# yimin-pan/hair-gs

Measured on AMD Instinct MI355X. Metric: train_iters_per_sec, higher is better.
Workload: dtype f32; 1 GPU; north_star: 100000 strand-Gaussians, 32 views @ 1920x1080, 1 view(s)/GPU/optimizer step (1 views/step), RGB+mask+orientation raster fwd+bwd + L1/DSSIM/mask/orientation/smoothness losses + Adam; gaussians=100000, views=32, width=1920, height=1080, parallelism=view-parallel x1, views_per_optimizer_step=1, forward_mode=async-capacity, dispatch=hip-graph replay, optimizer_steps_per_graph_launch=8, adam_in_backward_lanes=True, raster_passes_per_iter=1

## Files before the change

### hair-gs_amd/csrc/hgs_api.hip

```cpp
#include <stdarg.h>
#include <stdio.h>
#include <string.h>

#include "hgs_common.h"
#include "hgs_prologue.h"

static thread_local char g_err[512] = "";

void hgs_set_error(const char* fmt, ...) {
  va_list ap;
  va_start(ap, fmt);
  vsnprintf(g_err, sizeof(g_err), fmt, ap);
  va_end(ap);
}

#include <vector>
namespace {
struct ProfRec { hipEvent_t a, b; int id; };
bool g_prof_on = false;
std::vector<ProfRec> g_prof_log;
std::vector<hipEvent_t> g_prof_pool;
hipEvent_t g_prof_open = nullptr;
int g_prof_open_id = -1;
const char* kKernelNames[HGS_K_COUNT] = {"preprocess_fwd_kernel", "scan_kernel", "scatter_kernel", "sort_tiles_kernel",
// ... 215 lines not shown
    if (!fused_scan) { hgs_set_error("hgs_params_forward_preprocess: the scan must be the scatter kernel's (sizes beyond its limits)"); return 1; }
    HgsStrandFusion fu = fusion ? *fusion : HgsStrandFusion{};
    if (!(fu.smooth_pairs && fu.n_smooth > 0 && fu.smooth_partials)) fu.n_smooth = 0;
    if (hgs_launch_param_preprocess_fwd(s, a, g, im, radii, *params, fu)) return 1;
  } else if (hgs_launch_preprocess_fwd(s, a, g, im, radii)) return 1;
  if (!fused_scan && hgs_launch_scan(s, P, T, g, im, max_rendered, a.row_runs)) return 1;
  if (num_rendered_host) {
    uint32_t r = 0;
    HGS_CHECK_HIP(hipMemcpyAsync(&r, im.status, sizeof(uint32_t), hipMemcpyDeviceToHost, s));
    HGS_CHECK_HIP(hipStreamSynchronize(s));
    *num_rendered_host = (int)r;
  }
  return 0;
}

int hgs_forward_render(void* stream, int P, int W, int H, int R_capacity, int n_extra, int flags, const float* bg,
                       const float* colors_precomp, const float* extra, void* geom_buf, void* binning_buf, void* image_buf,
                       float* out_color) {
  hipStream_t s = (hipStream_t)stream;
  if (check_aligned(image_buf, "image_buf")) return 1;
  if (!bg || !out_color) { hgs_set_error("null bg/out_color"); return 1; }
  if (n_extra != 0 && n_extra != 4) { hgs_set_error("n_extra must be 0 or 4 (got %d)", n_extra); return 1; }
  if (n_extra && P > 0 && (!extra || ((size_t)extra & 15))) { hgs_set_error("extra colours must be a 16-byte aligned [P,4] array"); return 1; }
  if ((flags & HGS_RECORDS_PACKED) && (flags & HGS_RECORDS_LAZY)) { hgs_set_error("HGS_RECORDS_PACKED and HGS_RECORDS_LAZY exclude each other"); return 1; }
  const int channels = 3 + n_extra;
  HgsImage im;
  hgs_image_carve((char*)image_buf, (size_t)W, (size_t)H, im, nullptr);
  HgsGeom g = {};
  HgsBinning b = {};
  if (P > 0) {
    if (check_aligned(geom_buf, "geom_buf")) return 1;
    hgs_geom_carve((char*)geom_buf, (size_t)P, g, nullptr);
    if (R_capacity > 0) {
      if (check_aligned(binning_buf, "binning_buf")) return 1;
      hgs_binning_carve((char*)binning_buf, (size_t)R_capacity, b, nullptr, channels);
      b.grec = g.grec;
      const long long tiles = (long long)((W + HGS_TILE - 1) / HGS_TILE) * ((H + HGS_TILE - 1) / HGS_TILE);
      b.lazy = (flags & HGS_RECORDS_LAZY) ? 1 : (flags & HGS_RECORDS_PACKED) ? 0 : ((long long)R_capacity >= (long long)HGS_LAZY_MIN_MEAN_LIST * tiles ? 1 : 0);
    }
    const float* feat = colors_precomp ? colors_precomp : g.rgb;
    if (hgs_launch_scatter(s, P, W, H, R_capacity > 0 ? R_capacity : 0, feat, extra, n_extra, g, im, b)) return 1;
  }
  if (hgs_launch_sort_tiles(s, W, H, R_capacity > 0 ? R_capacity : 0, n_extra, g, im, b)) return 1;
  return hgs_launch_blend_fwd(s, W, H, R_capacity > 0 ? R_capacity : 0, channels, bg, im, b, out_color);
}

#define HGS_RR_AUTO_RATIO 8

static int backward_impl(void* stream, int P, int D, int M, int R, int W, int H, int n_extra, int flags, const float* bg,
                         const float* means3D, const float* shs, const float* colors_precomp, const float* scales,
                         float scale_modifier, const float* rotations, const float* cov3D_precomp, const float* viewmatrix,
                         const float* projmatrix, const float* campos, float tan_fovx, float tan_fovy, const int* radii,
                         const void* geom_buf, const void* binning_buf, const void* image_buf,
                         const float* const* dL_dpix_planes, void* scratch, float* dL_dextra, float* dL_dmeans2D, float* dL_dconic,
                         float* dL_dopacity, float* dL_dcolors, float* dL_dmeans3D, float* dL_dcov3D, float* dL_dsh,
                         float* dL_dscales, float* dL_drotations, const HgsParamBackward* pb,
                         const HgsBlockPlan* plan = nullptr) {
  hipStream_t s = (hipStream_t)stream;
  if (n_extra != 0 && n_extra != 4) { hgs_set_error("n_extra must be 0 or 4 (got %d)", n_extra); return 1; }
// ... 328 lines not shown
```

### hair-gs_amd/csrc/hgs_blend.hip

```cpp
#include "hgs_common.h"

__device__ unsigned long long* g_wg_trace_fwd = nullptr;
__device__ unsigned long long* g_wg_trace_bwd = nullptr;
#ifndef HGS_WG_TRACE
#define HGS_WG_TRACE 0
#endif
struct WgTrace {
#if HGS_WG_TRACE
  unsigned long long* buf;
  __device__ WgTrace(unsigned long long* b) : buf(b ? b + 8 * (size_t)blockIdx.x : nullptr) { mark(0); }
  __device__ void mark(int k) const { if (buf && threadIdx.x == 0) buf[k] = __builtin_amdgcn_s_memrealtime(); }
  __device__ void item(int tile, uint32_t seg, uint32_t nseg, uint32_t len) const {
    if (buf && threadIdx.x == 0) buf[6] = (unsigned long long)tile | (unsigned long long)seg << 24 | (unsigned long long)nseg << 32 | (unsigned long long)len << 40;
  }
  __device__ void count(int k, unsigned v) const { if (buf && (threadIdx.x & 63) == 0) atomicAdd(&buf[k], (unsigned long long)v); }
  __device__ ~WgTrace() { mark(7); }
#else
  __device__ WgTrace(unsigned long long*) {}
  __device__ void mark(int) const {}
  __device__ void item(int, uint32_t, uint32_t, uint32_t) const {}
  __device__ void count(int, unsigned) const {}
#endif
};

// ... 173 lines not shown
        process(rb, eb);
        if (__ballot(T > 0.f) == 0ull) m = 0ull;
        if (m == 0ull) break;
      }
    }
    if (b + 1 < nb) {
      if (threadIdx.x < REC_BATCH * REC4) recs[cur ^ 1][threadIdx.x] = stage;
      const uint32_t wave_alive = __ballot(T > 0.f) != 0 ? 1u : 0u;
      if (lane == 0) alive[cur ^ 1][wave] = wave_alive;
    }
  }
}

template <int C>
__global__ __launch_bounds__(HGS_BLOCK) __attribute__((amdgpu_waves_per_eu(8))) void blend_fwd_kernel(HgsImage im, HgsBinning bn, int W, int H, int gx, uint32_t Rcap,
                                                              const float* __restrict__ bg, float* __restrict__ out_color) {
  constexpr int REC4 = Chan<C>::REC4;
  __shared__ float4 recs[2][REC_BATCH * REC4];
  __shared__ uint32_t alive[2][4];
  __shared__ uint32_t s_flag;
  BlendItem it;
  if (!blend_item(im, Rcap, it)) return;
  const int tile = it.tile;
  WgTrace _trace(g_wg_trace_fwd);
  _trace.item(tile, it.seg, it.nseg, it.e - it.s);
  const int tx = tile % gx, ty = tile / gx;
  const int wave = threadIdx.x >> 6, lane = threadIdx.x & 63;
  const int px = tx * HGS_TILE + (wave & 1) * 8 + (lane & 7);
  const int py = ty * HGS_TILE + (wave >> 1) * 8 + (lane >> 3);
  const bool inside = px < W && py < H;
  const float pxf = (float)px, pyf = (float)py;
  const uint32_t list0 = it.range.x;
  float acc[C];
#pragma unroll
  for (int k = 0; k < C; k++) acc[k] = 0.f;
  uint32_t last = 0;
  const size_t pix = (size_t)py * W + px, HW = (size_t)H * W;

  if (!it.split) {
    float T = inside ? 1.f : -1.f;
    fwd_walk<C>(bn, it.lazy, list0, tx, ty, 0u, it.e, recs, alive, pxf, pyf, wave, lane, T, acc, last);
    uint32_t wmax = last;
#pragma unroll
    for (int d = 32; d >= 1; d >>= 1) wmax = max(wmax, (uint32_t)__shfl_xor((int)wmax, d, 64));
    if (lane == 0 && wmax) atomicMax(&im.tile_maxc[tile], wmax);
    if (inside) {
      T = fabsf(T);
      im.final_T[pix] = T;
      im.n_contrib[pix] = last;
#pragma unroll
      for (int k = 0; k < C; k++) out_color[k * HW + pix] = acc[k] + T * bg[k];
    }
    return;
  }

  if (it.nseg == 2u) {
    if (it.seg == 1u) return;
    const uint32_t n = it.range.y - it.range.x;
    float T = inside ? 1.f : -1.f;
    fwd_walk<C>(bn, it.lazy, list0, tx, ty, 0u, it.e, recs, alive, pxf, pyf, wave, lane, T, acc, last);
    const size_t slot1 = ((size_t)it.w + 1) * HGS_BLOCK + threadIdx.x;
    bn.seg_T[slot1] = fabsf(T);
#pragma unroll
    for (int k = 0; k < C; k++) { bn.seg_C[((size_t)it.w * C + k) * HGS_BLOCK + threadIdx.x] = acc[k]; acc[k] = 0.f; }
    fwd_walk<C>(bn, it.lazy, list0, tx, ty, it.e, n, recs, alive, pxf, pyf, wave, lane, T, acc, last);
#pragma unroll
    for (int k = 0; k < C; k++) {
      bn.seg_C[(((size_t)it.w + 1) * C + k) * HGS_BLOCK + threadIdx.x] = acc[k];
      acc[k] += bn.seg_C[((size_t)it.w * C + k) * HGS_BLOCK + threadIdx.x];
      bn.seg_C[((size_t)it.w * C + k) * HGS_BLOCK + threadIdx.x] = acc[k];
    }
    uint32_t wmax = last;
#pragma unroll
    for (int d = 32; d >= 1; d >>= 1) wmax = max(wmax, (uint32_t)__shfl_xor((int)wmax, d, 64));
    if (lane == 0 && wmax) atomicMax(&im.tile_maxc[tile], wmax);
    if (inside) {
      T = fabsf(T);
      im.final_T[pix] = T;
      im.n_contrib[pix] = last;
#pragma unroll
      for (int k = 0; k < C; k++) out_color[k * HW + pix] = acc[k] + T * bg[k];
    }
    return;
  }

  const size_t slot = (size_t)it.w * HGS_BLOCK + threadIdx.x;
  const size_t slot0 = slot - (size_t)it.seg * HGS_BLOCK;
  float T = inside ? 1.f : -1.f;
  fwd_walk<C>(bn, it.lazy, list0, tx, ty, it.s, it.e, recs, alive, pxf, pyf, wave, lane, T, acc, last);
  const float P = inside ? fmaxf(T, 0.f) : -1.f;
// ... 96 lines not shown
        v[j][k] = mh - j >= 0 ? hgs_ld_agent(&bn.seg_C[((w0 + (size_t)(mh - j)) * C + k) * HGS_BLOCK + threadIdx.x]) : 0.f;
#pragma unroll
    for (int j = 0; j < FG; j++)
      if (mh - j >= 0) {
#pragma unroll
        for (int k = 0; k < C; k++) {
          if ((uint32_t)(mh - j) <= lastseg) acc[k] += v[j][k];
          bn.seg_C[((w0 + (size_t)(mh - j)) * C + k) * HGS_BLOCK + threadIdx.x] = acc[k];
        }
      }
  }
  uint32_t wmax = inside ? nc : 0u;
#pragma unroll
  for (int d = 32; d >= 1; d >>= 1) wmax = max(wmax, (uint32_t)__shfl_xor((int)wmax, d, 64));
  if (lane == 0 && wmax) atomicMax(&im.tile_maxc[tile], wmax);
  if (inside) {
    im.final_T[pix] = Tfin;
    im.n_contrib[pix] = nc;
#pragma unroll
    for (int k = 0; k < C; k++) out_color[k * HW + pix] = acc[k] + Tfin * bg[k];
  }
}

template <int C> struct PixGrad { const float* plane[C]; };

template <int C, bool BLACK>
__global__ __launch_bounds__(HGS_BLOCK) __attribute__((amdgpu_waves_per_eu(HGS_BWD_WAVES))) void blend_bwd_kernel(HgsImage im, HgsBinning bn, int W, int H, int gx,
                                                              uint32_t Rcap, const float* __restrict__ bg,
                                                              PixGrad<C> dL_dpix, float* __restrict__ inst_grad, int tag_rows) {
  constexpr int REC4 = Chan<C>::REC4, NPART = Chan<C>::NPART, NREG = Chan<C>::NREG, NV = 4 * NREG, ROW = Chan<C>::ROW;
// ... 166 lines not shown

}

extern "C" int hgs_debug_set_wg_trace(void* device_buf_fwd, void* device_buf_bwd) {
  HGS_CHECK_HIP(hipMemcpyToSymbol(HIP_SYMBOL(g_wg_trace_fwd), &device_buf_fwd, sizeof(void*)));
  HGS_CHECK_HIP(hipMemcpyToSymbol(HIP_SYMBOL(g_wg_trace_bwd), &device_buf_bwd, sizeof(void*)));
  return 0;
}

static inline unsigned blend_grid(int T, const HgsBinning& b) {
  const unsigned cap = (unsigned)HGS_SPLIT_CAPACITY(T);
  return (unsigned)T + (b.seg_cap < cap ? b.seg_cap : cap);
}

int hgs_launch_blend_fwd(hipStream_t s, int W, int H, int Rcap, int channels, const float* bg, const HgsImage& im,
                         const HgsBinning& b, float* out_color) {
  const int gx = (W + HGS_TILE - 1) / HGS_TILE, gy = (H + HGS_TILE - 1) / HGS_TILE;
  {
    HgsProfScope _prof(s, HGS_K_BLEND_FWD);
    if (channels == 3)
      hipLaunchKernelGGL(blend_fwd_kernel<3>, dim3(blend_grid(gx * gy, b)), dim3(HGS_BLOCK), 0, s, im, b, W, H, gx,
                         (uint32_t)Rcap, bg, out_color);
    else
      hipLaunchKernelGGL(blend_fwd_kernel<7>, dim3(blend_grid(gx * gy, b)), dim3(HGS_BLOCK), 0, s, im, b, W, H, gx,
                         (uint32_t)Rcap, bg, out_color);
  }
  HGS_CHECK_LAUNCH();
  return 0;
}

int hgs_launch_blend_bwd(hipStream_t s, int W, int H, int Rcap, int channels, const float* bg, const HgsImage& im,
                         const HgsBinning& b, const float* const* dL_dpix_planes, float* inst_grad, int tag_rows) {
  const int gx = (W + HGS_TILE - 1) / HGS_TILE, gy = (H + HGS_TILE - 1) / HGS_TILE;
  {
    HgsProfScope _prof(s, HGS_K_BLEND_BWD);
    if (channels == 3) {
      PixGrad<3> pg;
      for (int k = 0; k < 3; k++) pg.plane[k] = dL_dpix_planes[k];
      if (bg) hipLaunchKernelGGL((blend_bwd_kernel<3, false>), dim3(blend_grid(gx * gy, b)), dim3(HGS_BLOCK), 0, s, im, b, W, H, gx,
                                 (uint32_t)Rcap, bg, pg, inst_grad, tag_rows);
// ... 15 lines not shown
```

### hair-gs_amd/csrc/hgs_common.h

```cpp
#pragma once
#include <hip/hip_runtime.h>
#include <stdint.h>
#include <stddef.h>

#include "../../include/hgs.h"

#define HGS_BLOCK 256
#define HGS_WAVE 64
#define HGS_ALIGN 256

struct HgsRect {
  uint16_t x0, y0, x1, y1;
  uint32_t off;
  uint32_t pad;
};

struct HgsGeom {
  float* depths; uint8_t* clamped; float2* means2D; float* cov3D; float4* conic_opacity; float* rgb;
  uint32_t* tiles_touched; uint32_t* point_offsets; HgsRect* rect; uint32_t* block_sums;
  float4* grec;
};
struct HgsImage {
  float* final_T; uint32_t* n_contrib; uint2* ranges; uint32_t* tile_count; uint32_t* tile_cursor;
  int32_t* tile_delta;
  uint32_t* tile_maxc; uint32_t* status; uint32_t* tile_order; uint32_t* wl_exchange;
  uint32_t tile_mask;
  uint32_t* tile_done; unsigned long long* tile_prog; unsigned long long* tile_sortprog; uint32_t* sort_items;
};
struct HgsBinning {
  uint64_t* keys; uint32_t* point_list; float4* packed; uint32_t* inv; uint64_t* keys_sorted;
  float* seg_P;
  float* seg_T;
  float* seg_Tout;
  uint32_t* seg_last;
  float* seg_C;
  uint32_t seg_cap;
  const float4* grec;
  int lazy;
};
#ifndef HGS_LAZY_MIN_MEAN_LIST
#define HGS_LAZY_MIN_MEAN_LIST 128
#endif
// ... 84 lines not shown
  const HgsImageZero z = hgs_image_zero_layout(T);
  im.tile_mask = (uint32_t)(Tp - 1);
  hgs_carve(cur, im.tile_count, T);         if (offs) offs[HGS_IMG_TILE_COUNT] = (char*)im.tile_count - base;
  uint32_t* const zr = im.tile_count;
  im.tile_delta = (int32_t*)(zr + z.delta);
  im.tile_cursor = zr + z.cursor;           if (offs) offs[HGS_IMG_TILE_CURSOR] = (char*)im.tile_cursor - base;
  im.tile_maxc = zr + z.maxc;               if (offs) offs[HGS_IMG_TILE_MAXC] = (char*)im.tile_maxc - base;
  im.tile_done = zr + z.done;
  im.status = zr + z.status;                if (offs) offs[HGS_IMG_STATUS] = (char*)im.status - base;
  im.tile_prog = (unsigned long long*)(zr + z.prog);
  im.tile_sortprog = (unsigned long long*)(zr + z.sortprog);
  cur = (char*)(zr + z.words);
  hgs_carve(cur, im.sort_items, T);
  hgs_carve(cur, im.tile_order, T + HGS_SPLIT_CAPACITY(T));  if (offs) offs[HGS_IMG_TILE_ORDER] = (char*)im.tile_order - base;
  hgs_carve(cur, im.wl_exchange, HGS_WL_EXCHANGE_WORDS);
  return hgs_align_up((size_t)(cur - base)) + HGS_ALIGN;
}
static inline size_t hgs_binning_carve(char* base, size_t R, HgsBinning& b, size_t* offs, int channels = 3) {
  char* cur = base;
  hgs_carve(cur, b.keys, R);                                  if (offs) offs[HGS_BIN_KEYS] = (char*)b.keys - base;
  hgs_carve(cur, b.point_list, R);                            if (offs) offs[HGS_BIN_POINT_LIST] = (char*)b.point_list - base;
  hgs_carve(cur, b.packed, R * (channels <= 3 ? HGS_PACKED_FLOATS / 4 : 4) + 4);  if (offs) offs[HGS_BIN_PACKED] = (char*)b.packed - base;
  hgs_carve(cur, b.inv, R);                                   if (offs) offs[HGS_BIN_INV] = (char*)b.inv - base;
  hgs_carve(cur, b.keys_sorted, R);                           if (offs) offs[HGS_BIN_KEYS_TMP] = (char*)b.keys_sorted - base;
  b.seg_cap = hgs_seg_capacity(R);
  hgs_carve(cur, b.seg_P, (size_t)b.seg_cap * 256);
  hgs_carve(cur, b.seg_T, (size_t)b.seg_cap * 256);
  hgs_carve(cur, b.seg_Tout, (size_t)b.seg_cap * 256);
  hgs_carve(cur, b.seg_last, (size_t)b.seg_cap * 256);
  hgs_carve(cur, b.seg_C, (size_t)b.seg_cap * 256 * (channels <= 3 ? 3 : 7));
// ... 83 lines not shown
};
#ifndef HGS_FUSED_SCAN_MAX_P
#define HGS_FUSED_SCAN_MAX_P 0x7FFFFFFF
#endif
#define HGS_FUSED_SCAN_MAX_T 8192
int hgs_launch_preprocess_fwd(hipStream_t s, const HgsFwdArgs& a, const HgsGeom& g, const HgsImage& im, int* radii);
int hgs_launch_param_preprocess_fwd(hipStream_t s, const HgsFwdArgs& a, const HgsGeom& g, const HgsImage& im, int* radii,
                                    const HgsParamForward& pf, const HgsStrandFusion& fusion);
int hgs_param_forward_check(int P, const HgsParamForward* pf, bool one_launch, const char* who);
int hgs_launch_scan(hipStream_t s, int P, int T, const HgsGeom& g, const HgsImage& im, unsigned int* max_rendered, int row_runs = 0);
int hgs_launch_scatter(hipStream_t s, int P, int W, int H, int Rcap, const float* features, const float* extra, int n_extra,
                       const HgsGeom& g, const HgsImage& im, const HgsBinning& b);
int hgs_launch_sort_tiles(hipStream_t s, int W, int H, int Rcap, int n_extra, const HgsGeom& g, const HgsImage& im,
                          const HgsBinning& b);
int hgs_launch_blend_fwd(hipStream_t s, int W, int H, int Rcap, int channels, const float* bg, const HgsImage& im,
                         const HgsBinning& b, float* out_color);
int hgs_launch_blend_bwd(hipStream_t s, int W, int H, int Rcap, int channels, const float* bg, const HgsImage& im,
                         const HgsBinning& b, const float* const* dL_dpix_planes, float* inst_grad, int tag_rows = 0);
struct HgsBwdArgs {
  int P, D, M, W, H;
  const float *means3D, *shs, *colors_precomp, *scales, *rotations, *cov3D_precomp;
  const float *viewmatrix, *projmatrix, *campos;
  float scale_modifier, tan_fovx, tan_fovy;
  const int* radii;
  float *dL_dmeans2D, *dL_dconic, *dL_dopacity, *dL_dcolors, *dL_dmeans3D, *dL_dcov3D, *dL_dsh, *dL_dscales,
      *dL_drotations;
  int n_extra;
  float* dL_dextra;
  const float* row_sums;
  const float* row_partials;
};
// ... 97 lines not shown
```

### hair-gs_amd/diff_gaussian_rasterization/_C.py

```python
import contextlib
import ctypes as C
import os

import torch

import hgs_runtime as rt

IMAGE_PREZEROED = 2
COUNT_ROW_RUNS = 4
TILE_CULL = 8
RECORDS_PACKED, RECORDS_LAZY = 16, 32
ROWS_INLINE, ROWS_REDUCE = 64, 128
_state = {"async": False, "slack": 1.5, "cap": 0, "dirty": False, "cap_used": None,
          "max_R": {}, "last_exact_R": 0, "last_counts_clean": False,
          "cull": None, "row_reduce": None, "lazy_records": None, "row_runs": None}


class HgsCapacityOverflow(RuntimeError):
    pass


def bucket_capacity(n):
    n = int(n)
    if n <= 16:
# ... 41 lines not shown
    was = _state["row_runs"]
    _state["row_runs"] = None if mode is None else bool(mode)
    return was


def _row_runs_flag(P, use_async):
    mode = _pinned(_state["row_runs"], "HGS_ROW_RUNS")
    if mode is None:
        mode = (_state["cap"] if use_async else _state["last_exact_R"]) >= 8 * P
    return COUNT_ROW_RUNS if (mode and P > 0) else 0


def set_async(enabled=True, slack=1.5):
    _state["async"], _state["slack"] = bool(enabled), float(slack)
    _state["dirty"], _state["cap_used"] = False, None


@contextlib.contextmanager
def async_mode(enabled, slack=None):
    saved = {k: _state[k] for k in ("async", "slack", "dirty", "cap_used")}
    _state["async"], _state["slack"] = bool(enabled), _state["slack"] if slack is None else float(slack)
    try:
        yield
    finally:
        _state.update(saved)


def capacity():
    return _state["cap"]

# ... 66 lines not shown
    return _forward(background, means3D, colors, opacity, scales, rotations, scale_modifier, cov3D_precomp, viewmatrix,
                    projmatrix, tan_fovx, tan_fovy, image_height, image_width, sh, degree, campos, prefiltered, debug,
                    None, False)


def rasterize_gaussians_culled(background, means3D, colors, opacity, scales, rotations, scale_modifier, cov3D_precomp,
                               viewmatrix, projmatrix, tan_fovx, tan_fovy, image_height, image_width, sh, degree, campos,
                               prefiltered, debug):
    return _forward(background, means3D, colors, opacity, scales, rotations, scale_modifier, cov3D_precomp, viewmatrix,
                    projmatrix, tan_fovx, tan_fovy, image_height, image_width, sh, degree, campos, prefiltered, debug,
                    None, True)


def rasterize_gaussians_multi(background7, means3D, colors, extra4, opacity, scales, rotations, scale_modifier,
                              cov3D_precomp, viewmatrix, projmatrix, tan_fovx, tan_fovy, image_height, image_width, sh,
                              degree, campos, prefiltered, debug, image_buffer=None, hair=None):
    return _forward(background7, means3D, colors, opacity, scales, rotations, scale_modifier, cov3D_precomp, viewmatrix,
                    projmatrix, tan_fovx, tan_fovy, image_height, image_width, sh, degree, campos, prefiltered, debug,
                    extra4, True, image_buffer, None, hair)


class _ParamSource:

    def __init__(self, kind, fusion, fill, fuse, **inputs):
        self.params, self.fusion, self.fill, self.fuse = rt.ParamForward(kind=kind), fusion, fill, bool(fuse)
        self.inputs = {k: rt.require_gpu_tensor(t, k, torch.int64) if k == "endpoint_pairs" else _f32(t, k) for k, t in inputs.items()}
        for k, t in self.inputs.items():
            setattr(self.params, k, rt.ptr(t))


class HairSource(_ParamSource):

    def __init__(self, endpoints, pairs, width, factor, opacity_raw, mask_raw, fusion=None, fill=None, fuse=True):
        super().__init__(rt.PARAMS_HAIR, fusion, fill, fuse, endpoints=endpoints, endpoint_pairs=pairs, width=width,
# ... 11 lines not shown
def will_fuse_hair(W, H):
    return (_state["async"] and _state["cap"] > 0 and os.environ.get("HGS_FUSE_PREPROCESS", "1") != "0"
            and ((int(W) + 15) // 16) * ((int(H) + 15) // 16) <= rt.FUSED_PREPROCESS_MAX_TILES)


def rasterize_gaussians_prezeroed(background, means3D, colors, opacity, scales, rotations, scale_modifier, cov3D_precomp,
                                  viewmatrix, projmatrix, tan_fovx, tan_fovy, image_height, image_width, sh, degree, campos,
                                  image_buffer, max_rendered=None, hair=None):
    return _forward(background, means3D, colors, opacity, scales, rotations, scale_modifier, cov3D_precomp, viewmatrix,
                    projmatrix, tan_fovx, tan_fovy, image_height, image_width, sh, degree, campos, False, False,
                    None, True, image_buffer, max_rendered, hair)


def _forward(background, means3D, colors, opacity, scales, rotations, scale_modifier, cov3D_precomp, viewmatrix,
             projmatrix, tan_fovx, tan_fovy, image_height, image_width, sh, degree, campos, prefiltered, debug, extra4,
             cull, image_buffer=None, max_rendered=None, hair=None):
    if means3D.ndim != 2 or means3D.shape[1] != 3:
        raise RuntimeError("means3D must have dimensions (num_points, 3)")
    L = rt.lib()
    means3D = rt.require_gpu_tensor(means3D, "means3D", torch.float32)
    dev = means3D.device
    P, H, W = means3D.shape[0], int(image_height), int(image_width)
    M = sh.shape[1] if (sh is not None and sh.numel() != 0) else 0
    n_ch = 3 if extra4 is None else 7
    extra_ = None if extra4 is None else rt.require_gpu_tensor(extra4, "extra4", torch.float32)
    out_color = torch.empty((n_ch, H, W), dtype=torch.float32, device=dev)
    radii = torch.empty((P,), dtype=torch.int32, device=dev)
    u8 = dict(dtype=torch.uint8, device=dev)
    geom = torch.empty((L.hgs_geom_bytes(P),), **u8)
    cull = _state["cull"] if _state["cull"] is not None else cull
    flags = int(bool(prefiltered)) | (TILE_CULL if cull else 0)
    if image_buffer is not None:
        if image_buffer.numel() != L.hgs_image_bytes(W, H) or image_buffer.dtype != torch.uint8 or image_buffer.device != dev:
            raise RuntimeError("image_buffer: need a uint8 tensor of hgs_image_bytes(W, H) on the inputs' device")
        img, flags = image_buffer, flags | IMAGE_PREZEROED
    else:
        img = torch.empty((L.hgs_image_bytes(W, H),), **u8)
    bg = _f32(background, "bg")
    colors_, opacity_, scales_, rots_, cov_, sh_ = (_f32(colors, "colors_precomp"), _f32(opacity, "opacities"),
                                                     _f32(scales, "scales"), _f32(rotations, "rotations"),
                                                     _f32(cov3D_precomp, "cov3D_precomp"), _f32(sh, "sh"))
# ... 25 lines not shown
            rt.check(L.hgs_forward_preprocess(stream, P, int(degree), M, W, H, rt.ptr(means3D), rt.ptr(sh_), rt.ptr(colors_),
                                              rt.ptr(opacity_), rt.ptr(scales_), float(scale_modifier), rt.ptr(rots_),
                                              rt.ptr(cov_), rt.ptr(view), rt.ptr(proj), rt.ptr(cam), float(tan_fovx),
                                              float(tan_fovy), flags, rt.ptr(geom), rt.ptr(img),
                                              rt.ptr(radii), None if use_async else C.addressof(n_host), mr_))
        if P > 0:
            _state["last_counts_clean"] = bool(use_async and ((W + 15) // 16) * ((H + 15) // 16) <= rt.FUSED_PREPROCESS_MAX_TILES)
        if use_async:
            R = _state["cap"]
        else:
            R = int(n_host.value)
            _state["last_exact_R"] = R
            if _state["async"]:
                raise_capacity(R)
        binning = torch.empty((L.hgs_binning_bytes(R, n_ch),), **u8)
        rt.check(L.hgs_forward_render(stream, P, W, H, R, n_ch - 3, _records_flags(), rt.ptr(bg), rt.ptr(colors_),
                                      rt.ptr(extra_), rt.ptr(geom), rt.ptr(binning), rt.ptr(img), rt.ptr(out_color)))
        if use_async and max_rendered is None:
            _mark_pending(R)
        if debug:
            torch.cuda.synchronize(dev)
    return R, out_color, radii, geom, binning, img


def _scratch(nbytes, dev):
    buf = torch.empty((nbytes,), dtype=torch.uint8, device=dev)
    if os.environ.get("HGS_POISON_SCRATCH") == "1" and nbytes >= 4:
        buf[:nbytes // 4 * 4].view(torch.float32).fill_(float("nan"))
    return buf


def _backward(n_extra, background, means3D, radii, colors, scales, rotations, scale_modifier, cov3D_precomp, viewmatrix,
# ... 81 lines not shown
```

### hair-gs_amd/hgs_runtime/__init__.py

```python
import ctypes as C
import os
import subprocess

import numpy as np

_PKG_ROOT = os.path.dirname(os.path.dirname(os.path.abspath(__file__)))
LIB_PATH = os.environ.get("HGS_LIB") or os.path.join(_PKG_ROOT, "libhgs.so")
CSRC = os.path.join(_PKG_ROOT, "csrc")
_lib = None

vp, ci, cf, sz = C.c_void_p, C.c_int, C.c_float, C.c_size_t

SIGNATURES = {
    "hgs_abi_version": (ci, []),
    "hgs_last_error": (C.c_char_p, []),
    "hgs_geom_bytes": (sz, [ci]),
    "hgs_image_bytes": (sz, [ci, ci]),
    "hgs_binning_bytes": (sz, [ci, ci]),
    "hgs_backward_scratch_bytes": (sz, [ci, ci, ci]),
    "hgs_forward_preprocess": (ci, [vp, ci, ci, ci, ci, ci, vp, vp, vp, vp, vp, cf, vp, vp, vp, vp, vp, cf, cf, ci,
                                    vp, vp, vp, vp, vp]),
    "hgs_forward_render": (ci, [vp, ci, ci, ci, ci, ci, ci, vp, vp, vp, vp, vp, vp, vp]),
    "hgs_backward": (ci, [vp, ci, ci, ci, ci, ci, ci, ci, ci, vp, vp, vp, vp, vp, cf, vp, vp, vp, vp, vp, cf, cf, vp, vp, vp,
                          vp, vp, vp, vp, vp, vp, vp, vp, vp, vp, vp, vp, vp]),
    "hgs_param_backward_bytes": (sz, []),
    "hgs_backward_multi_params": (ci, [vp, ci, ci, ci, ci, ci, ci, ci, vp, vp, vp, vp, vp, vp, vp, vp, cf, cf, vp, vp, vp, vp, vp,
                                       vp, vp, vp]),
    "hgs_block_plan_bytes": (sz, []),
    "hgs_backward_multi_params_planned": (ci, [vp, ci, ci, ci, ci, ci, ci, ci, vp, vp, vp, vp, vp, vp, vp, vp, cf, cf, vp, vp, vp, vp,
                                               vp, vp, vp, vp, vp]),
    "hgs_hair_endpoint_gather": (ci, [vp, ci, vp, vp, vp, vp, vp]),
    "hgs_mark_visible": (ci, [vp, ci, vp, vp, vp, vp]),
    "hgs_dist2_scratch_bytes": (sz, [ci]),
    "hgs_dist2": (ci, [vp, ci, vp, vp, vp, sz]),
    "hgs_ssim_l1_scratch_floats": (sz, [ci, ci, ci]),
    "hgs_ssim_l1_num_blocks": (ci, [ci, ci, ci]),
    "hgs_ssim_l1_forward": (ci, [vp, ci, ci, ci, vp, vp, vp, vp, vp]),
# ... 93 lines not shown
    "hgs_raster_count": (ci, [vp, ci, ci, ci, ci, vp, C.c_longlong, vp, ci, vp, vp, vp]),
    "hgs_raster_fill": (ci, [vp, ci, ci, ci, ci, vp, C.c_longlong, vp, ci, vp, vp, vp, vp, vp]),
    "hgs_raster_resolve": (ci, [vp, ci, ci, ci, ci, vp, vp, ci, vp, vp, vp, vp, vp, vp, vp, vp, vp, vp, vp]),
    "hgs_set_segment_policy": (ci, [ci, ci, ci]),
    "hgs_debug_set_wg_trace": (ci, [vp, vp]),
    "hgs_prof_enable": (ci, [ci]),
    "hgs_prof_bracket_overhead_ms": (C.c_double, []),
    "hgs_prof_collect": (ci, [vp, vp]),
    "hgs_prof_kernel_name": (C.c_char_p, [ci]),
    "hgs_geom_layout": (ci, [ci, vp]),
    "hgs_image_layout": (ci, [ci, ci, vp]),
    "hgs_binning_layout": (ci, [ci, vp]),
}
GEOM_FIELDS = ["depths", "clamped", "means2D", "cov3D", "conic_opacity", "rgb", "tiles_touched", "point_offsets", "rect",
               "block_sums"]
IMG_FIELDS = ["final_T", "n_contrib", "ranges", "tile_count", "tile_cursor", "tile_maxc", "status", "tile_order"]
BIN_FIELDS = ["keys", "point_list", "packed", "inv", "keys_sorted"]
PACKED_FLOATS = 12
INST_GRAD_FLOATS = 12


class HgsError(RuntimeError):
    pass


class ViewTargets(C.Structure):
    _fields_ = [("image", vp), ("float_mask", vp), ("orientation", vp), ("confidence", vp), ("mask", vp),
                ("viewmatrix", cf * 16), ("projmatrix", cf * 16), ("campos", cf * 3), ("mask_count", cf)]


class HeadParams(C.Structure):
# ... 301 lines not shown
```

### hair-gs_amd/hgs_runtime/strand_step.py

```python
import ctypes as C
import functools
import os
import math

import numpy as np
import torch

import hgs_runtime as rt
from hgs_runtime.fused import gaussian_window11

_SLOT_BYTES = C.sizeof(rt.ViewTargets)
_F_VIEW, _F_PROJ, _F_CAM = (rt.ViewTargets.viewmatrix.offset // 4, rt.ViewTargets.projmatrix.offset // 4,
                            rt.ViewTargets.campos.offset // 4)


class ViewTable:

    def __init__(self, cameras, device=None, targets=True):
        if len(cameras) == 0:
            raise rt.HgsError("ViewTable needs at least one camera")
        c0 = cameras[0]
        self.has_targets = bool(targets)
        if device is not None:
            self.device = torch.device(device)
# ... 38 lines not shown
            for k, v in enumerate(c.camera_center.detach().float().cpu().reshape(-1).tolist()):
                r.campos[k] = v
            self._keep.append(keep)
        host = torch.from_numpy(np.frombuffer(bytes(rows), dtype=np.uint8).copy())
        self.table = host.to(self.device)
        self.slot = torch.zeros(_SLOT_BYTES, dtype=torch.uint8, device=self.device)
        f = self.slot.view(torch.float32)
        self.viewmatrix, self.projmatrix, self.campos = f[_F_VIEW:_F_VIEW + 16], f[_F_PROJ:_F_PROJ + 16], f[_F_CAM:_F_CAM + 3]
        self._cameras = list(cameras)
        self.index = {id(c): i for i, c in enumerate(cameras)}
        self.n = len(cameras)
        self.current = -1
        self.queue = torch.zeros(rt.VIEW_QUEUE_MAX, dtype=torch.int32, device=self.device)
        self.queue_lr = torch.zeros((), dtype=torch.float32, device=self.device)
        self._image, self._zero, self._image_ready = None, None, False
        self._rider = None
        self.counts_clean = False
        self._fill_behind = False
        self.adam_prep = None

    def select(self, view, lr=0.0, lr_dst=None):
        if not 0 <= int(view) < self.n:
            raise rt.HgsError(f"view {view} outside the table (0..{self.n - 1})")
        with torch.cuda.device(self.device):
            rt.check(rt.lib().hgs_select_view(rt.current_stream(), self.table.data_ptr(), int(view), self.slot.data_ptr(),
                                              float(lr), None if lr_dst is None else lr_dst.data_ptr()))
        self.current = int(view)
        self._rider = None

    def _image_zero_range(self, behind_counts=False):
# ... 60 lines not shown
        self.counts_clean = True

    def ensure_counts_clean(self):
        if self.counts_clean or self._image is None:
            return
        (p0, _), (p1, _) = self._image_zero_range(False), self._image_zero_range(True)
        off = p0 - self._image.data_ptr()
        self._image[off:off + (p1 - p0)].zero_()
        self.counts_clean = True

    def take_image(self):
        if not self._image_ready:
            return None
        self._image_ready = False
        return self._image

    def graph_bind(self, cuda_graph, count=1):
        nodes, tags, n = (C.c_void_p * count)(), (C.c_float * count)(), C.c_int(0)
        rt.check(rt.lib().hgs_graph_find_prologues(C.c_void_p(int(cuda_graph.raw_cuda_graph())), count, nodes, tags, C.addressof(n)))
        order = sorted(range(n.value), key=lambda i: tags[i])
        if n.value != count or (count > 1 and [int(tags[i]) for i in order] != list(range(count))):
            raise rt.HgsError(f"graph_bind: expected {count} tagged prologue nodes, found {n.value} with tags {[tags[i] for i in order]}")
        return (cuda_graph, [nodes[i] for i in order], self._fill_behind)

    def graph_set(self, binding, view, lr=0.0, lr_dst=None, k=0):
        if not 0 <= int(view) < self.n:
            raise rt.HgsError(f"view {view} outside the table (0..{self.n - 1})")
        graph, nodes, behind = binding
        zp, zb = self._image_zero_range(behind)
        rt.check(rt.lib().hgs_graph_set_prologue(C.c_void_p(int(graph.raw_cuda_graph_exec())), C.c_void_p(nodes[k]),
# ... 97 lines not shown
    p.n_smooth = int(n_smooth)
    p.cos_threshold = float(np.cos(threshold_deg * np.pi / 180))
    p.eps = float(eps)
    p.n_endpoints = int(n_endpoints)
    return p


def _raster_head_forward(step, xyz, scale, quat, opacity, extra4, shs, endpoints, smooth_idx, smooth_partials, n_endpoints,
                         hair=None):
    from diff_gaussian_rasterization import _C as raster
    g, vt, hp, L = step.gaussians, step.views, step.head, rt.lib()
    dev = xyz.device
    f32 = dict(dtype=torch.float32, device=dev)
    empty = step.empty
    own_image = vt.take_image()
    R, planes, radii, geom, binning, img = raster.rasterize_gaussians_multi(
        step.bg7, xyz, empty, extra4, opacity, scale, quat, 1.0, empty, vt.viewmatrix, vt.projmatrix, vt.tanfovx,
        vt.tanfovy, vt.H, vt.W, shs, g.active_sh_degree, vt.campos, False, False, image_buffer=own_image, hair=hair)
    if own_image is not None and xyz.shape[0] > 0:
        vt.counts_clean = raster.last_counts_clean()
    hp.n_endpoints = n_endpoints
    if step.skip_unread_blocks:
        if step._tile_maxc_offset is None:
            step._tile_maxc_offset = rt.layout("image", vt.W, vt.H)["tile_maxc"]
        hp.tile_used = img.data_ptr() + step._tile_maxc_offset
        hp.tiles_x, hp.tiles_y = (vt.W + 15) // 16, (vt.H + 15) // 16
    else:
        hp.tile_used = None
    scratch = torch.empty((L.hgs_loss_head_scratch_floats(C.byref(hp)),), **f32)
    out = torch.empty((rt.HEAD_NOUT,), **f32)
    d_extra = torch.empty((4, vt.H, vt.W), **f32) if (step.one_pass_pixels and vt.has_mask) else None
    if step.poison_unwritten and d_extra is not None:
        d_extra.fill_(float("nan"))
# ... 467 lines not shown
```

### include/hgs.h

```cpp
#ifndef HGS_H_INCLUDED
#define HGS_H_INCLUDED

#include <stddef.h>
#include <stdint.h>

#ifdef __cplusplus
extern "C" {
#endif

#define HGS_ABI_VERSION 15
#define HGS_TILE 16

int hgs_abi_version(void);
const char* hgs_last_error(void);

size_t hgs_geom_bytes(int P);
size_t hgs_image_bytes(int W, int H);
size_t hgs_binning_bytes(int R, int channels);
size_t hgs_backward_scratch_bytes(int P, int R, int channels);

#define HGS_IMAGE_PREZEROED 2
#define HGS_COUNT_ROW_RUNS 4
#define HGS_TILE_CULL 8
#define HGS_WAIT_TIMED_OUT 0xFFFFFFFFu
int hgs_forward_preprocess(void* stream, int P, int D, int M, int W, int H,
                           const float* means3D, const float* shs, const float* colors_precomp,
                           const float* opacities, const float* scales, float scale_modifier,
                           const float* rotations, const float* cov3D_precomp,
                           const float* viewmatrix, const float* projmatrix, const float* campos,
                           float tan_fovx, float tan_fovy, int prefiltered,
                           void* geom_buf, void* image_buf, int* radii, int* num_rendered_host,
                           unsigned int* max_rendered);

#define HGS_RECORDS_PACKED 16
#define HGS_RECORDS_LAZY 32
int hgs_forward_render(void* stream, int P, int W, int H, int R_capacity, int n_extra, int flags,
                       const float* bg, const float* colors_precomp, const float* extra,
                       void* geom_buf, void* binning_buf, void* image_buf, float* out_color);

#define HGS_ROWS_INLINE 64
#define HGS_ROWS_REDUCE 128
int hgs_backward(void* stream, int P, int D, int M, int R, int W, int H, int n_extra, int flags, const float* bg,
                 const float* means3D, const float* shs, const float* colors_precomp,
                 const float* scales, float scale_modifier, const float* rotations,
                 const float* cov3D_precomp, const float* viewmatrix, const float* projmatrix,
                 const float* campos, float tan_fovx, float tan_fovy, const int* radii,
                 const void* geom_buf, const void* binning_buf, const void* image_buf,
                 const float* const* dL_dpix_planes, void* scratch, float* dL_dextra,
                 float* dL_dmeans2D, float* dL_dconic, float* dL_dopacity, float* dL_dcolors,
                 float* dL_dmeans3D, float* dL_dcov3D, float* dL_dsh, float* dL_dscales,
                 float* dL_drotations);

int hgs_mark_visible(void* stream, int P, const float* means3D, const float* viewmatrix,
// ... 349 lines not shown
int hgs_field_solve(void* stream, int nx, int ny, int nz, const long long* acc, double* dir, double* conf);
int hgs_strand_trace(void* stream, int S, const double* roots, const double* p0, const double* dir, const double* conf, double ox,
                     double oy, double oz, double h, int nx, int ny, int nz, double step, int max_steps, double cos_max, double min_conf,
                     int max_gap, double* joints, int* count, int* reason);

int hgs_field_fill(void* stream, int nx, int ny, int nz, const unsigned char* kind, const int* free_index, int F, double* a, double* b,
                   int sweeps);

int hgs_set_segment_policy(int min_len, int max_len, int target_segments);
int hgs_debug_set_wg_trace(void* device_buf_fwd, void* device_buf_bwd);

enum { HGS_GEOM_DEPTHS = 0, HGS_GEOM_CLAMPED, HGS_GEOM_MEANS2D, HGS_GEOM_COV3D, HGS_GEOM_CONIC_OPACITY,
       HGS_GEOM_RGB, HGS_GEOM_TILES_TOUCHED, HGS_GEOM_POINT_OFFSETS, HGS_GEOM_RECT, HGS_GEOM_BLOCK_SUMS,
       HGS_GEOM_NFIELDS };
enum { HGS_IMG_FINAL_T = 0, HGS_IMG_N_CONTRIB, HGS_IMG_RANGES, HGS_IMG_TILE_COUNT, HGS_IMG_TILE_CURSOR,
       HGS_IMG_TILE_MAXC, HGS_IMG_STATUS, HGS_IMG_TILE_ORDER, HGS_IMG_NFIELDS };
enum { HGS_BIN_KEYS = 0, HGS_BIN_POINT_LIST, HGS_BIN_PACKED, HGS_BIN_INV, HGS_BIN_KEYS_TMP, HGS_BIN_NFIELDS };
int hgs_geom_layout(int P, size_t* offsets );
int hgs_image_layout(int W, int H, size_t* offsets );
int hgs_binning_layout(int R, size_t* offsets );

#define HGS_STATUS_WORDS 16
#define HGS_PACKED_FLOATS 12
#define HGS_INST_GRAD_FLOATS 12

#ifdef __cplusplus
}
#endif
#endif
```

Measured before the change: 4306 iters/s.

## Skip rewriting background-only tiles in a persistent forward render target

Adds a per-tile epoch array to the image buffer and a persistent output tensor per view table, so empty tiles that were already filled with the same background in a prior render return early instead of rewriting final_T, n_contrib and colour pixels. An epoch is issued per background tensor, and any tile that becomes non-empty or split resets its epoch to zero. This saves memory bandwidth on empty tiles. In exchange it adds an epoch read and write per tile and keeps a persistent 7-plane target, and it depends on the image buffer and output not being modified between renders.

```diff
diff --git a/hair-gs_amd/csrc/hgs_api.hip b/hair-gs_amd/csrc/hgs_api.hip
--- a/hair-gs_amd/csrc/hgs_api.hip
+++ b/hair-gs_amd/csrc/hgs_api.hip
@@ -1,6 +1,8 @@
 #include <stdarg.h>
 #include <stdio.h>
 #include <string.h>
+
+#include <atomic>
 
 #include "hgs_common.h"
 #include "hgs_prologue.h"
@@ -253,9 +255,23 @@
   return 0;
 }
 
+unsigned int hgs_new_target_epoch(void) {
+  static std::atomic<unsigned int> next{1u};
+  unsigned int e = next.fetch_add(1u, std::memory_order_relaxed);
+  while (e == 0u) e = next.fetch_add(1u, std::memory_order_relaxed);
+  return e;
+}
+
 int hgs_forward_render(void* stream, int P, int W, int H, int R_capacity, int n_extra, int flags, const float* bg,
                        const float* colors_precomp, const float* extra, void* geom_buf, void* binning_buf, void* image_buf,
                        float* out_color) {
+  return hgs_forward_render_target(stream, P, W, H, R_capacity, n_extra, flags, bg, colors_precomp, extra, geom_buf, binning_buf,
+                                   image_buf, out_color, 0u);
+}
+
+int hgs_forward_render_target(void* stream, int P, int W, int H, int R_capacity, int n_extra, int flags, const float* bg,
+                              const float* colors_precomp, const float* extra, void* geom_buf, void* binning_buf, void* image_buf,
+                              float* out_color, unsigned int target_epoch) {
   hipStream_t s = (hipStream_t)stream;
   if (check_aligned(image_buf, "image_buf")) return 1;
   if (!bg || !out_color) { hgs_set_error("null bg/out_color"); return 1; }
@@ -281,7 +297,7 @@
     if (hgs_launch_scatter(s, P, W, H, R_capacity > 0 ? R_capacity : 0, feat, extra, n_extra, g, im, b)) return 1;
   }
   if (hgs_launch_sort_tiles(s, W, H, R_capacity > 0 ? R_capacity : 0, n_extra, g, im, b)) return 1;
-  return hgs_launch_blend_fwd(s, W, H, R_capacity > 0 ? R_capacity : 0, channels, bg, im, b, out_color);
+  return hgs_launch_blend_fwd(s, W, H, R_capacity > 0 ? R_capacity : 0, channels, bg, im, b, out_color, (uint32_t)target_epoch);
 }
 
 #define HGS_RR_AUTO_RATIO 8
diff --git a/hair-gs_amd/csrc/hgs_blend.hip b/hair-gs_amd/csrc/hgs_blend.hip
--- a/hair-gs_amd/csrc/hgs_blend.hip
+++ b/hair-gs_amd/csrc/hgs_blend.hip
@@ -211,7 +211,8 @@
 
 template <int C>
 __global__ __launch_bounds__(HGS_BLOCK) __attribute__((amdgpu_waves_per_eu(8))) void blend_fwd_kernel(HgsImage im, HgsBinning bn, int W, int H, int gx, uint32_t Rcap,
-                                                              const float* __restrict__ bg, float* __restrict__ out_color) {
+                                                              const float* __restrict__ bg, float* __restrict__ out_color,
+                                                              uint32_t target_epoch) {
   constexpr int REC4 = Chan<C>::REC4;
   __shared__ float4 recs[2][REC_BATCH * REC4];
   __shared__ uint32_t alive[2][4];
@@ -235,12 +236,15 @@
   const size_t pix = (size_t)py * W + px, HW = (size_t)H * W;
 
   if (!it.split) {
+    const bool empty = it.e == 0u;
+    if (empty && target_epoch != 0u && im.tile_bg_epoch[tile] == target_epoch) return;
     float T = inside ? 1.f : -1.f;
     fwd_walk<C>(bn, it.lazy, list0, tx, ty, 0u, it.e, recs, alive, pxf, pyf, wave, lane, T, acc, last);
     uint32_t wmax = last;
 #pragma unroll
     for (int d = 32; d >= 1; d >>= 1) wmax = max(wmax, (uint32_t)__shfl_xor((int)wmax, d, 64));
     if (lane == 0 && wmax) atomicMax(&im.tile_maxc[tile], wmax);
+    if (threadIdx.x == 0) im.tile_bg_epoch[tile] = empty ? target_epoch : 0u;
     if (inside) {
       T = fabsf(T);
       im.final_T[pix] = T;
@@ -271,6 +275,7 @@
 #pragma unroll
     for (int d = 32; d >= 1; d >>= 1) wmax = max(wmax, (uint32_t)__shfl_xor((int)wmax, d, 64));
     if (lane == 0 && wmax) atomicMax(&im.tile_maxc[tile], wmax);
+    if (threadIdx.x == 0) im.tile_bg_epoch[tile] = 0u;
     if (inside) {
       T = fabsf(T);
       im.final_T[pix] = T;
@@ -397,6 +402,7 @@
 #pragma unroll
   for (int d = 32; d >= 1; d >>= 1) wmax = max(wmax, (uint32_t)__shfl_xor((int)wmax, d, 64));
   if (lane == 0 && wmax) atomicMax(&im.tile_maxc[tile], wmax);
+  if (threadIdx.x == 0) im.tile_bg_epoch[tile] = 0u;
   if (inside) {
     im.final_T[pix] = Tfin;
     im.n_contrib[pix] = nc;
@@ -593,16 +599,16 @@
 }
 
 int hgs_launch_blend_fwd(hipStream_t s, int W, int H, int Rcap, int channels, const float* bg, const HgsImage& im,
-                         const HgsBinning& b, float* out_color) {
+                         const HgsBinning& b, float* out_color, uint32_t target_epoch) {
   const int gx = (W + HGS_TILE - 1) / HGS_TILE, gy = (H + HGS_TILE - 1) / HGS_TILE;
   {
     HgsProfScope _prof(s, HGS_K_BLEND_FWD);
     if (channels == 3)
       hipLaunchKernelGGL(blend_fwd_kernel<3>, dim3(blend_grid(gx * gy, b)), dim3(HGS_BLOCK), 0, s, im, b, W, H, gx,
-                         (uint32_t)Rcap, bg, out_color);
+                         (uint32_t)Rcap, bg, out_color, target_epoch);
     else
       hipLaunchKernelGGL(blend_fwd_kernel<7>, dim3(blend_grid(gx * gy, b)), dim3(HGS_BLOCK), 0, s, im, b, W, H, gx,
-                         (uint32_t)Rcap, bg, out_color);
+                         (uint32_t)Rcap, bg, out_color, target_epoch);
   }
   HGS_CHECK_LAUNCH();
   return 0;
diff --git a/hair-gs_amd/csrc/hgs_common.h b/hair-gs_amd/csrc/hgs_common.h
--- a/hair-gs_amd/csrc/hgs_common.h
+++ b/hair-gs_amd/csrc/hgs_common.h
@@ -26,6 +26,7 @@
   uint32_t* tile_maxc; uint32_t* status; uint32_t* tile_order; uint32_t* wl_exchange;
   uint32_t tile_mask;
   uint32_t* tile_done; unsigned long long* tile_prog; unsigned long long* tile_sortprog; uint32_t* sort_items;
+  uint32_t* tile_bg_epoch;
 };
 struct HgsBinning {
   uint64_t* keys; uint32_t* point_list; float4* packed; uint32_t* inv; uint64_t* keys_sorted;
@@ -140,6 +141,7 @@
   hgs_carve(cur, im.sort_items, T);
   hgs_carve(cur, im.tile_order, T + HGS_SPLIT_CAPACITY(T));  if (offs) offs[HGS_IMG_TILE_ORDER] = (char*)im.tile_order - base;
   hgs_carve(cur, im.wl_exchange, HGS_WL_EXCHANGE_WORDS);
+  hgs_carve(cur, im.tile_bg_epoch, T);                       if (offs) offs[HGS_IMG_TILE_BG_EPOCH] = (char*)im.tile_bg_epoch - base;
   return hgs_align_up((size_t)(cur - base)) + HGS_ALIGN;
 }
 static inline size_t hgs_binning_carve(char* base, size_t R, HgsBinning& b, size_t* offs, int channels = 3) {
@@ -253,7 +255,7 @@
 int hgs_launch_sort_tiles(hipStream_t s, int W, int H, int Rcap, int n_extra, const HgsGeom& g, const HgsImage& im,
                           const HgsBinning& b);
 int hgs_launch_blend_fwd(hipStream_t s, int W, int H, int Rcap, int channels, const float* bg, const HgsImage& im,
-                         const HgsBinning& b, float* out_color);
+                         const HgsBinning& b, float* out_color, uint32_t target_epoch = 0u);
 int hgs_launch_blend_bwd(hipStream_t s, int W, int H, int Rcap, int channels, const float* bg, const HgsImage& im,
                          const HgsBinning& b, const float* const* dL_dpix_planes, float* inst_grad, int tag_rows = 0);
 struct HgsBwdArgs {
diff --git a/hair-gs_amd/diff_gaussian_rasterization/_C.py b/hair-gs_amd/diff_gaussian_rasterization/_C.py
--- a/hair-gs_amd/diff_gaussian_rasterization/_C.py
+++ b/hair-gs_amd/diff_gaussian_rasterization/_C.py
@@ -79,6 +79,10 @@
 def set_async(enabled=True, slack=1.5):
     _state["async"], _state["slack"] = bool(enabled), float(slack)
     _state["dirty"], _state["cap_used"] = False, None
+
+
+def is_async():
+    return _state["async"]
 
 
 @contextlib.contextmanager
@@ -175,10 +179,10 @@
 
 def rasterize_gaussians_multi(background7, means3D, colors, extra4, opacity, scales, rotations, scale_modifier,
                               cov3D_precomp, viewmatrix, projmatrix, tan_fovx, tan_fovy, image_height, image_width, sh,
-                              degree, campos, prefiltered, debug, image_buffer=None, hair=None):
+                              degree, campos, prefiltered, debug, image_buffer=None, hair=None, out=None, target_epoch=0):
     return _forward(background7, means3D, colors, opacity, scales, rotations, scale_modifier, cov3D_precomp, viewmatrix,
                     projmatrix, tan_fovx, tan_fovy, image_height, image_width, sh, degree, campos, prefiltered, debug,
-                    extra4, True, image_buffer, None, hair)
+                    extra4, True, image_buffer, None, hair, out, target_epoch)
 
 
 class _ParamSource:
@@ -220,7 +224,7 @@
 
 def _forward(background, means3D, colors, opacity, scales, rotations, scale_modifier, cov3D_precomp, viewmatrix,
              projmatrix, tan_fovx, tan_fovy, image_height, image_width, sh, degree, campos, prefiltered, debug, extra4,
-             cull, image_buffer=None, max_rendered=None, hair=None):
+             cull, image_buffer=None, max_rendered=None, hair=None, out=None, target_epoch=0):
     if means3D.ndim != 2 or means3D.shape[1] != 3:
         raise RuntimeError("means3D must have dimensions (num_points, 3)")
     L = rt.lib()
@@ -230,7 +234,15 @@
     M = sh.shape[1] if (sh is not None and sh.numel() != 0) else 0
     n_ch = 3 if extra4 is None else 7
     extra_ = None if extra4 is None else rt.require_gpu_tensor(extra4, "extra4", torch.float32)
-    out_color = torch.empty((n_ch, H, W), dtype=torch.float32, device=dev)
+    target_epoch = int(target_epoch) if os.environ.get("HGS_BG_TILE_EPOCH", "1") != "0" else 0
+    if out is not None:
+        if (tuple(out.shape) != (n_ch, H, W) or out.dtype != torch.float32 or out.device != dev or not out.is_contiguous()):
+            raise RuntimeError(f"out: need a contiguous float32 [{n_ch}, H, W] tensor on the inputs' device")
+        out_color = out
+    else:
+        out_color = torch.empty((n_ch, H, W), dtype=torch.float32, device=dev)
+    if target_epoch != 0 and (out is None or image_buffer is None):
+        raise RuntimeError("target_epoch names a persistent (image_buffer, out) pair: both must be given")
     radii = torch.empty((P,), dtype=torch.int32, device=dev)
     u8 = dict(dtype=torch.uint8, device=dev)
     geom = torch.empty((L.hgs_geom_bytes(P),), **u8)
@@ -286,8 +298,9 @@
             if _state["async"]:
                 raise_capacity(R)
         binning = torch.empty((L.hgs_binning_bytes(R, n_ch),), **u8)
-        rt.check(L.hgs_forward_render(stream, P, W, H, R, n_ch - 3, _records_flags(), rt.ptr(bg), rt.ptr(colors_),
-                                      rt.ptr(extra_), rt.ptr(geom), rt.ptr(binning), rt.ptr(img), rt.ptr(out_color)))
+        rt.check(L.hgs_forward_render_target(stream, P, W, H, R, n_ch - 3, _records_flags(), rt.ptr(bg), rt.ptr(colors_),
+                                             rt.ptr(extra_), rt.ptr(geom), rt.ptr(binning), rt.ptr(img), rt.ptr(out_color),
+                                             target_epoch))
         if use_async and max_rendered is None:
             _mark_pending(R)
         if debug:
diff --git a/hair-gs_amd/hgs_runtime/__init__.py b/hair-gs_amd/hgs_runtime/__init__.py
--- a/hair-gs_amd/hgs_runtime/__init__.py
+++ b/hair-gs_amd/hgs_runtime/__init__.py
@@ -21,6 +21,8 @@
     "hgs_forward_preprocess": (ci, [vp, ci, ci, ci, ci, ci, vp, vp, vp, vp, vp, cf, vp, vp, vp, vp, vp, cf, cf, ci,
                                     vp, vp, vp, vp, vp]),
     "hgs_forward_render": (ci, [vp, ci, ci, ci, ci, ci, ci, vp, vp, vp, vp, vp, vp, vp]),
+    "hgs_forward_render_target": (ci, [vp, ci, ci, ci, ci, ci, ci, vp, vp, vp, vp, vp, vp, vp, C.c_uint]),
+    "hgs_new_target_epoch": (C.c_uint, []),
     "hgs_backward": (ci, [vp, ci, ci, ci, ci, ci, ci, ci, ci, vp, vp, vp, vp, vp, cf, vp, vp, vp, vp, vp, cf, cf, vp, vp, vp,
                           vp, vp, vp, vp, vp, vp, vp, vp, vp, vp, vp, vp, vp]),
     "hgs_param_backward_bytes": (sz, []),
@@ -144,7 +146,7 @@
 }
 GEOM_FIELDS = ["depths", "clamped", "means2D", "cov3D", "conic_opacity", "rgb", "tiles_touched", "point_offsets", "rect",
                "block_sums"]
-IMG_FIELDS = ["final_T", "n_contrib", "ranges", "tile_count", "tile_cursor", "tile_maxc", "status", "tile_order"]
+IMG_FIELDS = ["final_T", "n_contrib", "ranges", "tile_count", "tile_cursor", "tile_maxc", "status", "tile_order", "tile_bg_epoch"]
 BIN_FIELDS = ["keys", "point_list", "packed", "inv", "keys_sorted"]
 PACKED_FLOATS = 12
 INST_GRAD_FLOATS = 12
diff --git a/hair-gs_amd/hgs_runtime/strand_step.py b/hair-gs_amd/hgs_runtime/strand_step.py
--- a/hair-gs_amd/hgs_runtime/strand_step.py
+++ b/hair-gs_amd/hgs_runtime/strand_step.py
@@ -76,6 +76,7 @@
         self.queue = torch.zeros(rt.VIEW_QUEUE_MAX, dtype=torch.int32, device=self.device)
         self.queue_lr = torch.zeros((), dtype=torch.float32, device=self.device)
         self._image, self._zero, self._image_ready = None, None, False
+        self._target, self._target_epoch, self._target_bg = None, 0, None
         self._rider = None
         self.counts_clean = False
         self._fill_behind = False
@@ -166,6 +167,16 @@
             return None
         self._image_ready = False
         return self._image
+
+    def take_target(self, bg7):
+        if self._image is None:
+            raise rt.HgsError("take_target: the table has no image buffer yet (prologue() creates it)")
+        if self._target is None:
+            self._target = torch.empty((7, self.H, self.W), dtype=torch.float32, device=self.device)
+            self._target_bg = None
+        if self._target_bg is not bg7:
+            self._target_bg, self._target_epoch = bg7, int(rt.lib().hgs_new_target_epoch())
+        return self._target, self._target_epoch
 
     def graph_bind(self, cuda_graph, count=1):
         nodes, tags, n = (C.c_void_p * count)(), (C.c_float * count)(), C.c_int(0)
@@ -293,9 +304,12 @@
     f32 = dict(dtype=torch.float32, device=dev)
     empty = step.empty
     own_image = vt.take_image()
+    target, epoch = (vt.take_target(step.bg7) if (own_image is not None and raster.is_async())
+                     else (None, 0))
     R, planes, radii, geom, binning, img = raster.rasterize_gaussians_multi(
         step.bg7, xyz, empty, extra4, opacity, scale, quat, 1.0, empty, vt.viewmatrix, vt.projmatrix, vt.tanfovx,
-        vt.tanfovy, vt.H, vt.W, shs, g.active_sh_degree, vt.campos, False, False, image_buffer=own_image, hair=hair)
+        vt.tanfovy, vt.H, vt.W, shs, g.active_sh_degree, vt.campos, False, False, image_buffer=own_image, hair=hair,
+        out=target, target_epoch=epoch)
     if own_image is not None and xyz.shape[0] > 0:
         vt.counts_clean = raster.last_counts_clean()
     hp.n_endpoints = n_endpoints
diff --git a/include/hgs.h b/include/hgs.h
--- a/include/hgs.h
+++ b/include/hgs.h
@@ -37,6 +37,10 @@
 int hgs_forward_render(void* stream, int P, int W, int H, int R_capacity, int n_extra, int flags,
                        const float* bg, const float* colors_precomp, const float* extra,
                        void* geom_buf, void* binning_buf, void* image_buf, float* out_color);
+int hgs_forward_render_target(void* stream, int P, int W, int H, int R_capacity, int n_extra, int flags,
+                              const float* bg, const float* colors_precomp, const float* extra,
+                              void* geom_buf, void* binning_buf, void* image_buf, float* out_color, unsigned int target_epoch);
+unsigned int hgs_new_target_epoch(void);
 
 #define HGS_ROWS_INLINE 64
 #define HGS_ROWS_REDUCE 128
@@ -416,7 +420,7 @@
        HGS_GEOM_RGB, HGS_GEOM_TILES_TOUCHED, HGS_GEOM_POINT_OFFSETS, HGS_GEOM_RECT, HGS_GEOM_BLOCK_SUMS,
        HGS_GEOM_NFIELDS };
 enum { HGS_IMG_FINAL_T = 0, HGS_IMG_N_CONTRIB, HGS_IMG_RANGES, HGS_IMG_TILE_COUNT, HGS_IMG_TILE_CURSOR,
-       HGS_IMG_TILE_MAXC, HGS_IMG_STATUS, HGS_IMG_TILE_ORDER, HGS_IMG_NFIELDS };
+       HGS_IMG_TILE_MAXC, HGS_IMG_STATUS, HGS_IMG_TILE_ORDER, HGS_IMG_TILE_BG_EPOCH, HGS_IMG_NFIELDS };
 enum { HGS_BIN_KEYS = 0, HGS_BIN_POINT_LIST, HGS_BIN_PACKED, HGS_BIN_INV, HGS_BIN_KEYS_TMP, HGS_BIN_NFIELDS };
 int hgs_geom_layout(int P, size_t* offsets );
 int hgs_image_layout(int W, int H, size_t* offsets );
```

After: 4296 iters/s. About the same (-0.2%).
